# KLab/YAIK

Hardware: AMD Instinct MI355X
Metric: Mpix/s tile encode (alpha reject + 7 gradient passes + 8x8 range quant), 8K RGBA (higher is better)
Workload: dtype u8/int32 (+f32 mode-selection sums)

## Files before the change

### yaik_amd/csrc/yk_stages.hip

```cpp
#include "yk_common.h"
#ifdef YK_TEST_HOOKS
#include "../../include/yaik_hip_test.h"
#endif
#include "yk_device.h"

typedef int yk_i4 __attribute__((ext_vector_type(4)));
#ifndef YK_ALPHA_WAVES
#define YK_ALPHA_WAVES 3
#endif
__global__ __launch_bounds__(64 * YK_ALPHA_WAVES, 4) void yk_alpha_kernel(const int32_t* __restrict__ alpha0, int strideElems, int w, int h, int y0,
                                                      uint8_t* __restrict__ keep0, int mtW, int mtH, unsigned long long planeStride,
                                                      unsigned long long keepStride, yk_i4* __restrict__ unitBox0, unsigned total) {
    const int lane = threadIdx.x & 63;
    const int vecPerRow = w >> 2;
    const int nSeg = (vecPerRow + 63) >> 6;
    const int nUnits = nSeg * ((mtH + YK_ALPHA_R - 1) / YK_ALPHA_R);
    const unsigned uu = blockIdx.x * YK_ALPHA_WAVES + (threadIdx.x >> 6);
    if (uu >= total) return;
    const int f = (int)(uu / (unsigned)nUnits), u = (int)(uu - (unsigned)f * (unsigned)nUnits);
    const int32_t* alpha = alpha0 + (size_t)f * planeStride;
    uint8_t* keep = keep0 + (size_t)f * keepStride;
    const int tyU = u / nSeg, seg = u - tyU * nSeg, ty0 = tyU * YK_ALPHA_R;
    const int xv = seg * 64 + lane;
    const bool inX = xv < vecPerRow;
    const bool tileLane = (lane & 3) == 0;
    const int tx = xv >> 2;
    const int xvc = min(xv, vecPerRow - 1);
    uint32_t nzBits = 0, undBits = 0, rowsLeft = 0;
    {
        yk_i4 p[YK_ALPHA_R][2];
#pragma unroll
        for (int r = 0; r < YK_ALPHA_R; r++) {
            const int yA = min((ty0 + r) * 16, h - 1), yB = min(yA + 15, h - 1);
            p[r][0] = __builtin_nontemporal_load(reinterpret_cast<const yk_i4*>(alpha + (size_t)yA * strideElems + (size_t)xvc * 4));
            p[r][1] = __builtin_nontemporal_load(reinterpret_cast<const yk_i4*>(alpha + (size_t)yB * strideElems + (size_t)xvc * 4));
        }
#pragma unroll
        for (int r = 0; r < YK_ALPHA_R; r++) {
            const bool on = inX && (ty0 + r) * 16 < h;
            const yk_i4 o = p[r][0] | p[r][1];
            const bool nz = ((o.x | o.y | o.z | o.w) != 0) & on;
            const unsigned long long pb = __ballot(nz);
            const bool und = on && ((pb >> (lane & ~3)) & 0xFULL) == 0;
            nzBits |= (nz ? 1u : 0u) << r; undBits |= (und ? 1u : 0u) << r;
            if (__ballot(und) != 0) rowsLeft |= 1u << r;
        }
    }
    while (rowsLeft) {
        const int rA = __ffs((int)rowsLeft) - 1; rowsLeft &= rowsLeft - 1;
        const bool two = rowsLeft != 0;
        const int rB = two ? __ffs((int)rowsLeft) - 1 : rA; rowsLeft &= rowsLeft - 1;
        yk_i4 a[2][14];
#pragma unroll
        for (int j = 0; j < 2; j++) {
            const int r = j ? rB : rA, ty = ty0 + r;
            const bool und = (j == 0 || two) && ((undBits >> r) & 1u) != 0;
            const int32_t* col = alpha + (size_t)(ty * 16) * strideElems + (size_t)xv * 4;
#pragma unroll
            for (int k = 0; k < 14; k++) {
                a[j][k] = (yk_i4){0, 0, 0, 0};
                if (und && ty * 16 + 1 + k < h) a[j][k] = __builtin_nontemporal_load(reinterpret_cast<const yk_i4*>(col + (size_t)(1 + k) * strideElems));
            }
        }
#pragma unroll
        for (int j = 0; j < 2; j++) {
            int m = 0;
#pragma unroll
            for (int k = 0; k < 14; k++) m |= a[j][k].x | a[j][k].y | a[j][k].z | a[j][k].w;
            nzBits |= (m != 0 ? 1u : 0u) << (j ? rB : rA);
        }
    }
    int colLo = 0x7FFFFFFF, colHi = -1, rowLo = 0x7FFFFFFF, rowHi = -1;
#pragma unroll
    for (int r = 0; r < YK_ALPHA_R; r++) {
        const int ty = ty0 + r;
        if (ty >= mtH) break;
        const unsigned long long b = __ballot(((nzBits >> r) & 1u) != 0);
        const bool kept = ((b >> (lane & ~3)) & 0xFULL) != 0;
        if (tileLane && tx < mtW) keep[(size_t)ty * mtW + tx] = kept ? 1 : 0;
        const unsigned long long kb64 = __ballot(tileLane && kept && tx < mtW);
        if (kb64) {
            colLo = min(colLo, seg * 16 + ((__ffsll((long long)kb64) - 1) >> 2));
            colHi = max(colHi, seg * 16 + ((63 - __clzll((long long)kb64)) >> 2));
            rowLo = min(rowLo, ty); rowHi = max(rowHi, ty);
        }
    }
    if (lane == 0) {
        const bool any = colHi >= 0;
        unitBox0[(size_t)f * nUnits + u] = any ? (yk_i4){colLo * 16, y0 + rowLo * 16, colHi * 16 + 16, y0 + rowHi * 16 + 16} : (yk_i4){9999999, 9999999, -1, -1};
    }
}

__global__ __launch_bounds__(256) void yk_alpha_box_kernel(const yk_i4* __restrict__ unitBox0, int nUnits, int32_t* __restrict__ bounds) {
    __shared__ yk_i4 s_box[4];
    const int lane = threadIdx.x & 63, wv = threadIdx.x >> 6;
    const yk_i4* ub = unitBox0 + (size_t)blockIdx.x * nUnits;
    int x0 = 9999999, gy0 = 9999999, x1 = -1, gy1 = -1;
    for (int base = 0; base < nUnits; base += 256 * 16) {
        yk_i4 v[16];
#pragma unroll
        for (int j = 0; j < 16; j++) v[j] = ub[min(base + j * 256 + (int)threadIdx.x, nUnits - 1)];
#pragma unroll
        for (int j = 0; j < 16; j++) { x0 = min(x0, v[j].x); gy0 = min(gy0, v[j].y); x1 = max(x1, v[j].z); gy1 = max(gy1, v[j].w); }
    }
#pragma unroll
    for (int d = 1; d < 64; d <<= 1) {
        x0 = min(x0, __shfl_xor(x0, d)); x1 = max(x1, __shfl_xor(x1, d));
        gy0 = min(gy0, __shfl_xor(gy0, d)); gy1 = max(gy1, __shfl_xor(gy1, d));
    }
    if (lane == 0) s_box[wv] = (yk_i4){x0, gy0, x1, gy1};
    __syncthreads();
    if (threadIdx.x == 0) {
#pragma unroll
        for (int k = 1; k < 4; k++) { x0 = min(x0, s_box[k].x); gy0 = min(gy0, s_box[k].y); x1 = max(x1, s_box[k].z); gy1 = max(gy1, s_box[k].w); }
        *reinterpret_cast<yk_i4*>(bounds + (size_t)blockIdx.x * 16 + 8) = (yk_i4){x0, gy0, x1, gy1};
    }
}

__global__ void yk_alpha_publish_kernel(int32_t* __restrict__ bounds, int srcOff, int fullW, int fullH) {
    bounds += (size_t)blockIdx.x * 16;
    const int b0 = bounds[srcOff], b1 = bounds[srcOff + 1], b2 = bounds[srcOff + 2], b3 = bounds[srcOff + 3];
    bounds[0] = b0; bounds[1] = b1; bounds[2] = b2; bounds[3] = b3;
    bounds[4] = (b0 == 0 && b1 == 0 && b2 == fullW && b3 == fullH) ? 1 : 0;
}

#define YK_SCAN_TILE 1024

__global__ __launch_bounds__(1024) void yk_scan1_kernel(const uint8_t* __restrict__ tileCount, size_t T8, uint32_t* __restrict__ blockCnt) {
    __shared__ uint32_t s_tmp[32];
    const size_t i = (size_t)blockIdx.x * YK_SCAN_TILE + threadIdx.x;
    const uint32_t c = (i < T8) ? tileCount[i] : 0;
    uint32_t tot2, totN;
    yk_block_exscan(c ? 1u : 0u, s_tmp, &tot2);
    yk_block_exscan(c, s_tmp, &totN);
    if (threadIdx.x == 0) { blockCnt[(size_t)blockIdx.x * 2] = totN; blockCnt[(size_t)blockIdx.x * 2 + 1] = tot2; }
}

__device__ __forceinline__ void yk_scan2_body(uint32_t* __restrict__ blockCnt, uint32_t* __restrict__ blockSums, int nBlocks, uint32_t* __restrict__ totals, uint32_t* s_tmp) {
    uint32_t baseN = 0, baseD = 0;
    for (int start = 0; start < nBlocks; start += 1024) {
        const int i = start + threadIdx.x;
        const uint32_t n = i < nBlocks ? blockCnt[i * 2] : 0, d = i < nBlocks ? blockCnt[i * 2 + 1] : 0;
        uint32_t totN, totD;
        const uint32_t en = yk_block_exscan(n, s_tmp, &totN);
        const uint32_t ed = yk_block_exscan(d, s_tmp, &totD);
        if (i < nBlocks) {
            blockSums[i * 2] = baseN + en; blockSums[i * 2 + 1] = baseD + ed;
            blockCnt[i * 2] = 0; blockCnt[i * 2 + 1] = 0;
        }
        baseN += totN; baseD += totD;
    }
    if (threadIdx.x < 3) { totals[threadIdx.x * 2] = baseD; totals[threadIdx.x * 2 + 1] = baseN; }
}
__global__ __launch_bounds__(1024) void yk_scan2_kernel(uint32_t* __restrict__ blockCnt, uint32_t* __restrict__ blockSums, int nBlocks,
                                                        uint32_t* __restrict__ totals, unsigned long long blockNStride) {
    __shared__ uint32_t s_tmp[32];
    yk_scan2_body(blockCnt + (size_t)blockIdx.x * blockNStride, blockSums + (size_t)blockIdx.x * blockNStride, nBlocks, totals + (size_t)blockIdx.x * 8, s_tmp);
}

__global__ __launch_bounds__(1024) void yk_scan1r_kernel(const uint32_t* __restrict__ runSums, unsigned long long runStride, int nRuns,
                                                         uint32_t* __restrict__ blockCnt, unsigned long long blockNStride, int nBlocks,
                                                         const uint8_t* __restrict__ bm0b, unsigned long long bm0bStride, uint8_t* __restrict__ bitmap0,
                                                         unsigned long long bitmap0Stride, int nB64) {
    const size_t f = blockIdx.y;
    const int g = (int)blockIdx.x * 1024 + (int)threadIdx.x;
    if (runSums) {
        const uint4* rs4 = reinterpret_cast<const uint4*>(runSums + f * runStride);
        const int n4 = (nRuns + 3) >> 2;
        const uint4 v = g < n4 ? rs4[g] : make_uint4(0u, 0u, 0u, 0u);
        uint32_t acc = v.x + v.y + v.z + v.w;
        acc += __shfl_xor(acc, 16, 32); acc += __shfl_xor(acc, 8, 32); acc += __shfl_xor(acc, 4, 32); acc += __shfl_xor(acc, 2, 32); acc += __shfl_xor(acc, 1, 32);
        const int blk = g >> 5;
        if ((threadIdx.x & 31) == 0 && blk < nBlocks) {
            uint2* dst = reinterpret_cast<uint2*>(blockCnt + f * blockNStride) + blk;
            *dst = make_uint2(16u * (acc & 0xFFFFu), acc >> 16);
        }
    }
    if (g < nB64) {
        const uint32_t b = reinterpret_cast<const uint32_t*>(bm0b + f * bm0bStride)[g];
        uint16_t* dst = reinterpret_cast<uint16_t*>(bitmap0 + f * bitmap0Stride);
        dst[g] = (uint16_t)((b & 0xFu) | ((b >> 4) & 0xF0u) | ((b >> 8) & 0xF00u) | ((b >> 12) & 0xF000u));
        if (g == nB64 - 1 && (nB64 & 1)) dst[nB64] = 0;
    }
}

struct __attribute__((aligned(8))) YkPiece16 { uint32_t a, b, c, d; };
__global__ __launch_bounds__(256) void yk_pack_kernel(const uint8_t* __restrict__ tileCount, const uint16_t* __restrict__ tileDef, const uint2* __restrict__ tileInfo,
                                                      const uint8_t* __restrict__ slots, size_t T8, const uint32_t* __restrict__ blockSums, int nBlocks,
                                                      uint16_t* __restrict__ defsOut, uint32_t* __restrict__ nibOut, size_t nibStrideWords, YkFrameStrides fs,
                                                      const uint32_t* __restrict__ blockCnt, uint32_t* __restrict__ totals) {
    __shared__ uint32_t s_wave[4];
    __shared__ unsigned long long s_pre;
    __shared__ uint32_t s_off[YK_SCAN_TILE];
    __shared__ uint8_t s_cnt[YK_SCAN_TILE];
    {
        const size_t f = blockIdx.z;
        tileCount += f * fs.tileCount; tileDef += f * fs.tileDef; slots += f * fs.slots; blockSums += f * fs.blockN;
        if (tileInfo) tileInfo += f * fs.tileInfo;
        defsOut += f * fs.defsOut; nibOut += f * (fs.nibOut / 4);
        if (blockCnt) { blockCnt += f * fs.blockN; totals += f * 8; }
    }
    const int lane = threadIdx.x & 63, wave = threadIdx.x >> 6;
    const size_t i0 = (size_t)blockIdx.x * YK_SCAN_TILE, i = i0 + (size_t)threadIdx.x * 4;
    uint32_t c[4] = {0, 0, 0, 0}, d01[4] = {0, 0, 0, 0}, d2[4] = {0, 0, 0, 0};
    if (tileInfo && i + 4 <= T8) {
        const uint4 r0 = reinterpret_cast<const uint4*>(tileInfo + i)[0], r1 = reinterpret_cast<const uint4*>(tileInfo + i)[1];
        d01[0] = r0.x; c[0] = r0.y >> 16; d2[0] = r0.y & 0xFFFFu; d01[1] = r0.z; c[1] = r0.w >> 16; d2[1] = r0.w & 0xFFFFu;
        d01[2] = r1.x; c[2] = r1.y >> 16; d2[2] = r1.y & 0xFFFFu; d01[3] = r1.z; c[3] = r1.w >> 16; d2[3] = r1.w & 0xFFFFu;
    } else {
#pragma unroll
        for (int j = 0; j < 4; j++) {
            if (i + j >= T8) continue;
            if (tileInfo) { const uint2 ti = tileInfo[i + j]; c[j] = ti.y >> 16; d01[j] = ti.x; d2[j] = ti.y & 0xFFFFu; }
            else { c[j] = tileCount[i + j]; if (c[j]) { d01[j] = (uint32_t)tileDef[i + j] | ((uint32_t)tileDef[T8 + i + j] << 16); d2[j] = tileDef[2 * T8 + i + j]; } }
        }
    }
    if (blockCnt && wave == 3) {
        unsigned long long acc = 0;
        for (int k = lane; k < (int)blockIdx.x; k += 64) { const uint2 v = reinterpret_cast<const uint2*>(blockCnt)[k]; acc += ((unsigned long long)v.y << 32) | v.x; }
#pragma unroll
        for (int d = 1; d < 64; d <<= 1) acc += __shfl_xor(acc, d);
        if (lane == 0) s_pre = acc;
    }
    uint32_t w[4], mine = 0;
#pragma unroll
    for (int j = 0; j < 4; j++) { w[j] = mine; mine += c[j] | (c[j] ? 0x10000u : 0u); }
    uint32_t incl = mine;
#pragma unroll
    for (int d = 1; d < 64; d <<= 1) { const uint32_t o = __shfl_up(incl, d); if (lane >= d) incl += o; }
    if (lane == 63) s_wave[wave] = incl;
    __syncthreads();
    uint32_t front = incl - mine;
#pragma unroll
    for (int k = 0; k < 3; k++) if (k < wave) front += s_wave[k];
    uint32_t baseN, baseD;
    if (blockCnt) {
        baseN = (uint32_t)s_pre; baseD = (uint32_t)(s_pre >> 32);
        if (blockIdx.x == (unsigned)nBlocks - 1 && threadIdx.x < 3) {
            const uint2 v = reinterpret_cast<const uint2*>(blockCnt)[nBlocks - 1];
            totals[threadIdx.x * 2] = baseD + v.y; totals[threadIdx.x * 2 + 1] = baseN + v.x;
        }
    } else { baseN = blockSums[(size_t)blockIdx.x * 2]; baseD = blockSums[(size_t)blockIdx.x * 2 + 1]; }
#pragma unroll
    for (int j = 0; j < 4; j++) {
        const uint32_t e = front + w[j], en = e & 0xFFFFu, ed = e >> 16;
        s_off[threadIdx.x * 4 + j] = (baseN + en) >> 1;
        s_cnt[threadIdx.x * 4 + j] = (uint8_t)c[j];
        if (c[j]) { defsOut[baseD + ed] = (uint16_t)d01[j]; defsOut[T8 + baseD + ed] = (uint16_t)(d01[j] >> 16); defsOut[2 * T8 + baseD + ed] = (uint16_t)d2[j]; }
    }
    __syncthreads();
    const int half = threadIdx.x & 1;
#pragma unroll
    for (int p = 0; p < 3; p++) {
        uint8_t* out = reinterpret_cast<uint8_t*>(nibOut + (size_t)p * nibStrideWords);
#pragma unroll
        for (int it = 0; it < 8; it++) {
            const int t = it * 128 + (threadIdx.x >> 1);
            const size_t ti = i0 + t;
            const int left = (s_cnt[t] >> 1) - half * 16;
            const uint8_t* src = slots + ((size_t)p * T8 + ti) * YK_SLOT + half * 16;
            uint8_t* dst = out + s_off[t] + half * 16;
            if (left >= 16) { const uint4 v = *reinterpret_cast<const uint4*>(src); *reinterpret_cast<YkPiece16*>(dst) = YkPiece16{v.x, v.y, v.z, v.w}; }
            else if (left >= 8) *reinterpret_cast<uint2*>(dst) = *reinterpret_cast<const uint2*>(src);
        }
    }
}

static int (*g_crossCheckLauncher)(hipStream_t, const YkEncodeParams*) = nullptr;
#ifdef YK_TEST_HOOKS
extern "C" int yk_set_cross_check_launcher(void* fn) { g_crossCheckLauncher = reinterpret_cast<int (*)(hipStream_t, const YkEncodeParams*)>(fn); return YK_OK; }
#endif

int yk_launch_alpha(yk_ctx* c, bool batch) {
    const int F = batch ? c->nFrames : 1;
    const YkFrameView V = yk_frame(c, batch ? 0 : c->curFrame);
    const long long nUnits = (long long)yk_alpha_units(c->fullW, c->mtH);
    if (nUnits * F > 0x7FFFFFFFLL) return yk_fail(c, YK_ERR_BAD_ARG, "too many alpha work units for one launch");
    yk_i4* unitBox = reinterpret_cast<yk_i4*>(static_cast<int*>(c->img.alphaUnitBox));
    hipLaunchKernelGGL(yk_alpha_kernel, dim3((unsigned)((nUnits * F + YK_ALPHA_WAVES - 1) / YK_ALPHA_WAVES)), dim3(64 * YK_ALPHA_WAVES), 0, c->stream, V.plane[3], c->strideElems,
                       c->fullW, c->h, c->y0, V.keep, c->mtW, c->mtH, (unsigned long long)c->fs.plane, (unsigned long long)c->fs.keep, unitBox, (unsigned)(nUnits * F));
    hipLaunchKernelGGL(yk_alpha_box_kernel, dim3((unsigned)F), dim3(256), 0, c->stream, unitBox, (int)nUnits, V.bounds);
    YK_HIP(c, hipGetLastError());
    c->boundsOff = 8;
    return YK_OK;
}

int yk_launch_alpha_finish(yk_ctx* c, const int32_t* globalBBox) {
    if (globalBBox) {
        int32_t b[5] = { globalBBox[0], globalBBox[1], globalBBox[2], globalBBox[3], 0 };
        b[4] = (b[0] == 0 && b[1] == 0 && b[2] == c->fullW && b[3] == c->fullH) ? 1 : 0;
        YK_HIP(c, hipMemcpyAsync(yk_frame(c).bounds, b, sizeof b, hipMemcpyHostToDevice, c->stream));
        c->boundsOff = 0;
    }
    return YK_OK;
}

int yk_launch_encode(yk_ctx* c, int rejectFactor, int mode3BitOnly, int wantDst, bool batch) {
    const YkFrameView V = yk_frame(c, batch ? 0 : c->curFrame);
    YkEncodeParams P;
    for (int i = 0; i < 4; i++) P.plane[i] = V.plane[i];
    P.strideElems = c->strideElems; P.w = c->fullW; P.h = c->h; P.hAvail = c->h + c->halo; P.y0 = c->y0; P.fullH = c->fullH;
    P.rejectFactor = rejectFactor; P.startMode = mode3BitOnly ? 3 : 0; P.wantDst = wantDst; P.ablate = c->ablate;
    P.keep = (c->nPlanes == 4) ? V.keep : nullptr;
    P.bounds = (c->nPlanes == 4) ? V.bounds + c->boundsOff : nullptr;
    for (int i = 0; i < 7; i++) P.bitmap[i] = V.bitmap[i];
    P.coverage = V.coverage; P.tileDef = V.tileDef; P.tileCount = V.tileCount; P.slots = V.slots;
    P.blockCnt = c->kernelVersion == 2 ? V.blockCnt : nullptr;
    for (int i = 0; i < 3; i++) P.dst[i] = c->img.dst[i];
    P.tilesW = c->tilesW; P.tilesH = c->tilesH; P.mtW = c->mtW; P.mtH = c->mtH;
    P.xBB64 = (c->fullW + 63) / 64; P.yBB64 = (c->h + 63) / 64; P.xBB32 = (c->fullW + 31) / 32; P.yBB32 = (c->h + 31) / 32;
    P.nFrames = batch ? c->nFrames : 1; P.fs = c->fs;
    P.qtab = c->qtab;
    P.small = V.small;
    auto off = [&](const void* p) { return (uint32_t)(static_cast<const uint8_t*>(p) - V.small); };
    for (int i = 0; i < 7; i++) P.oBm[i] = off(V.bitmap[i]);
    P.oBm0b = off(V.bm0b); P.oCov = off(V.coverage); P.oInfo = off(V.tileInfo); P.oRun = off(V.runSums);
    P.divXBB64 = c->divXBB64; P.divNBf = c->divNBf;
    P.outTab = c->img.outTab; P.outFrame0 = batch ? 0u : (uint32_t)c->curFrame;
    P.pixCache = nullptr; c->pixCacheValid = false;
    if (c->pixCacheOn && !batch && c->kernelVersion == 2 && c->nFrames == 1) {
        if (!c->img.pixCache) YK_HIP(c, c->img.pixCache.alloc(c->stream, (size_t)P.xBB64 * 64 * ((size_t)(c->h + 15) / 16 * 16) / 4, 4096));
        P.pixCache = c->img.pixCache; c->pixCacheValid = true;
    }
    if (c->kernelVersion == 2) return yk_launch_encode2(c, P);
    if (batch) return yk_fail(c, YK_ERR_STATE, "batches need kernel version 2");
    if (c->nPlanes == 4) {
        hipLaunchKernelGGL(yk_alpha_publish_kernel, dim3(1), dim3(1), 0, c->stream, V.bounds, c->boundsOff, c->fullW, c->fullH);
        P.bounds = V.bounds;
    }
    if (!g_crossCheckLauncher) return yk_fail(c, YK_ERR_STATE, "kernel version 1 is not part of this library: register it with yk_set_cross_check_launcher");
    if (g_crossCheckLauncher(c->stream, &P) != 0) return yk_fail(c, YK_ERR_HIP, "cross-check kernel launch", hipGetLastError());
    return YK_OK;
}

int yk_launch_pack(yk_ctx* c, bool batch) {
    const size_t T8 = (size_t)c->tilesW * c->tilesH;
    const int nb = c->nScanBlocks, F = batch ? c->nFrames : 1;
    const YkFrameView V = yk_frame(c, batch ? 0 : c->curFrame);
    if (c->kernelVersion != 2) hipLaunchKernelGGL(yk_scan1_kernel, dim3(nb), dim3(1024), 0, c->stream, V.tileCount, T8, V.blockCnt);
    const bool v2 = c->kernelVersion == 2;
    const uint32_t* runSums = (v2 && (c->tilesW & 7) == 0) ? V.runSums : nullptr;
    const uint8_t* bm0b = v2 ? V.bm0b : nullptr;
    const uint2* tileInfo = v2 ? V.tileInfo : nullptr;
    const int nB64 = ((c->fullW + 63) / 64) * ((c->h + 63) / 64);
    if (v2) {
        const int nRuns = (int)((T8 + 7) / 8), n4 = (nRuns + 3) >> 2;
        const int items = runSums ? (n4 > nB64 ? n4 : nB64) : nB64;
        hipLaunchKernelGGL(yk_scan1r_kernel, dim3((unsigned)((items + 1023) / 1024), F), dim3(1024), 0, c->stream, runSums, (unsigned long long)c->fs.runSums, nRuns,
                           V.blockCnt, (unsigned long long)c->fs.blockN, nb, bm0b, (unsigned long long)c->fs.bm0b,
                           V.bitmap[0], (unsigned long long)c->fs.bitmap[0], nB64);
    }
    if (!runSums) hipLaunchKernelGGL(yk_scan2_kernel, dim3(F), dim3(1024), 0, c->stream, V.blockCnt, V.blockSums, nb, V.totals, (unsigned long long)c->fs.blockN);
    hipLaunchKernelGGL(yk_pack_kernel, dim3(nb, 1, F), dim3(256), 0, c->stream, V.tileCount, V.tileDef, tileInfo,
                       V.slots, T8, V.blockSums, nb, V.defsOut, reinterpret_cast<uint32_t*>(V.nibOut), c->nibStride / 4, c->fs,
                       runSums ? V.blockCnt : (const uint32_t*)nullptr, V.totals);
    YK_HIP(c, hipGetLastError());
    return YK_OK;
}

__global__ void yk_selftest_div_kernel(int* mismatches) {
    const int n = blockIdx.x, d = threadIdx.x + 1;
    const float fn = (float)n, fd = (float)d;
    const float ref = __fdiv_rn(fn, fd);
    const float got = yk_div_exact(fn, fd, __fdiv_rn(1.0f, fd));
    if (__float_as_uint(ref) != __float_as_uint(got)) atomicAdd(mismatches, 1);
}

__global__ void yk_selftest_scale_kernel(int* mismatches) {
    const int scale = blockIdx.x + 1, d8 = threadIdx.x;
    if (d8 < 32) return;
    const int dnum = (d8 - 32) * 127 + (scale - 1);
    const int ref = dnum / scale;
    const int got = __float2int_rz(((float)dnum + 0.5f) * __builtin_amdgcn_rcpf((float)scale));
    if (ref != got) atomicAdd(mismatches, 1);
}

__global__ void yk_selftest_r1div_kernel(int* mismatches) {
    const int n = blockIdx.x * 16 + (threadIdx.x >> 4), d0 = (threadIdx.x & 15) * 16;
    for (int k = 0; k < 16; k++) {
        const int d = d0 + k;
        if (d < 1 || d > 255) continue;
        const int got = __float2int_rz(((float)n + 0.5f) * __builtin_amdgcn_rcpf((float)d));
        if (got != n / d) atomicAdd(mismatches, 1);
    }
}

__global__ void yk_selftest_r1magic_kernel(int* mismatches) {
    const int delta = blockIdx.x, x = threadIdx.x;
    if (x > delta) return;
    for (int minCol = 0; minCol + delta <= 255; minCol++) {
        uint32_t A, B;
        yk_r1_magic(delta, minCol, &A, &B);
        const int v = minCol + x;
        int idx = 0;
        if (delta) { const int n = (v - minCol) * 15 + (delta >> 1) - 1; idx = n < 0 ? -1 : n / delta; }
        const uint32_t got = (__umul24((uint32_t)v, A) + B) >> 20;
        if (got != (uint32_t)(1 + idx)) atomicAdd(mismatches, 1);
    }
}

#ifdef YK_TEST_HOOKS
extern "C" int yk_selftest(yk_ctx* c, int which, int* result) {
    if (!c || !result) return YK_ERR_BAD_ARG;
    YK_HIP(c, hipSetDevice(c->device));
    YkBuf<int> d;
    YK_HIP(c, d.alloc(c->stream, 1));
    YK_HIP(c, hipMemsetAsync(d, 0, sizeof(int), c->stream));
    if (which == 0) hipLaunchKernelGGL(yk_selftest_div_kernel, dim3(256), dim3(256), 0, c->stream, d);
    else if (which == 1) hipLaunchKernelGGL(yk_selftest_scale_kernel, dim3(256), dim3(256), 0, c->stream, d);
    else if (which == 2) hipLaunchKernelGGL(yk_selftest_r1div_kernel, dim3(256), dim3(256), 0, c->stream, d);
    else if (which == 3) yk_selftest_qtab_launch(c, d);
    else if (which == 4) hipLaunchKernelGGL(yk_selftest_r1magic_kernel, dim3(256), dim3(256), 0, c->stream, d);
    else return yk_fail(c, YK_ERR_BAD_ARG, "unknown selftest");
    YK_HIP(c, hipMemcpyAsync(result, d, sizeof(int), hipMemcpyDeviceToHost, c->stream));
    YK_HIP(c, hipStreamSynchronize(c->stream));
    return YK_OK;
}
#endif
```

Measured before the change: 240,300.

## Compact coded tiles in pack kernel and batch slot loads for memory-level parallelism

The pack kernel now builds a compacted list of coded tiles in shared memory (offset plus tile index and count), so threads iterate only over real work items instead of every tile. Loads for several items are issued together before a waitcnt, then stored, to keep more memory requests in flight. Optional nontemporal load and store paths are added behind macros. Profiling scripts for the pack kernel are also added. The cost is more registers per thread and a loop over the compacted item list.

```diff
diff --git a/profiles/pack_in_flight/pack_frames.py b/profiles/pack_in_flight/pack_frames.py
--- /dev/null
+++ b/profiles/pack_in_flight/pack_frames.py
@@ -0,0 +1,26 @@
+import os, sys
+sys.path.insert(0, os.path.dirname(os.path.dirname(os.path.dirname(os.path.abspath(__file__)))))
+import torch
+from yaik_amd.encoder import HipTileEncoder
+
+reps, classes = int(sys.argv[1]), sys.argv[2:]
+W = 8192
+dev = "cuda"
+enc = HipTileEncoder(0)
+for name in classes:
+    if name == "noise":
+        g = torch.Generator(device=dev); g.manual_seed(1)
+        img = torch.randint(0, 256, (3, W, W), device=dev, generator=g)
+    elif name == "ramp":
+        x = torch.arange(W, device=dev, dtype=torch.int64)[None, :].expand(W, W)
+        y = torch.arange(W, device=dev, dtype=torch.int64)[:, None].expand(W, W)
+        img = torch.stack([(255 * x) // W, (255 * y) // W, (255 * (x + y)) // (2 * W)])
+    else:
+        raise SystemExit(f"unknown class {name}")
+    planes = img.to(torch.int32).contiguous()
+    enc.set_image(planes)
+    for _ in range(reps + 2):
+        enc.encode(3, False, False)
+    defs, _, nn = enc.range_streams(0)
+    print(f"class {name}: {nn} nibbles per plane, coded tiles {defs.size} of {W * W // 64}", flush=True)
+enc.close()
diff --git a/profiles/pack_in_flight/summarize.py b/profiles/pack_in_flight/summarize.py
--- /dev/null
+++ b/profiles/pack_in_flight/summarize.py
@@ -0,0 +1,48 @@
+import csv, glob, os, runpy, statistics, sys
+
+mode, d = sys.argv[1], sys.argv[2]
+S, E = (lambda r: int(r["Start_Timestamp"])), (lambda r: int(r["End_Timestamp"]))
+
+
+def kernel_rows(pattern):
+    rows = []
+    for f in glob.glob(f"{d}/**/*kernel_trace.csv", recursive=True):
+        rows += [r for r in csv.DictReader(open(f)) if pattern(r["Kernel_Name"])]
+    rows.sort(key=S)
+    return rows
+
+
+def line(label, us, mb):
+    med = statistics.median(us)
+    rate = f"  {mb:.1f} MB / median = {mb / med:.2f} TB/s" if mb else ""
+    print(f"{label}: yk_pack_kernel min {min(us):6.1f} us  median {med:6.1f} us  max {max(us):6.1f} us  ({len(us)} launches){rate}")
+
+
+if mode == "bench":
+    label, mb = sys.argv[3], float(sys.argv[4])
+    pack = kernel_rows(lambda n: "yk_pack_kernel" in n)
+    sel = pack[len(pack) // 4: len(pack) * 3 // 4]
+    line(label, [(E(r) - S(r)) / 1e3 for r in sel], mb)
+elif mode == "classes":
+    reps, classes = int(sys.argv[3]), [a.split(":") for a in sys.argv[4:]]
+    pack = kernel_rows(lambda n: "yk_pack_kernel" in n)
+    per = reps + 2
+    assert len(pack) == per * len(classes), (len(pack), per, classes)
+    for i, (name, mb) in enumerate(classes):
+        line(f"all-{name} 8192^2 RGB frame, alone", [(E(r) - S(r)) / 1e3 for r in pack[i * per + 2:(i + 1) * per]], float(mb))
+elif mode == "timeline":
+    sys.argv = [os.path.join(os.path.dirname(os.path.abspath(__file__)), "..", "event_chain", "summarize.py"), "timeline", d]
+    runpy.run_path(sys.argv[0], run_name="__main__")
+    rows = kernel_rows(lambda n: "yk_pack_kernel" in n or "encode2" in n)
+    fused = [r for r in rows if "encode2" in r["Kernel_Name"]]
+    lo, hi = S(fused[len(fused) // 4]), S(fused[len(fused) * 3 // 4])
+    st, en, dur = [], [], []
+    for r in rows:
+        if "yk_pack_kernel" not in r["Kernel_Name"] or not lo <= S(r) <= hi:
+            continue
+        other = min(fused, key=lambda f: abs(S(f) - S(r)))
+        st.append((S(r) - S(other)) / 1e3); en.append((E(r) - S(other)) / 1e3); dur.append((E(r) - S(r)) / 1e3)
+    print(f"\npack kernel, {len(st)} frames: starts {statistics.mean(st):+.1f} us (min {min(st):+.1f}, max {max(st):+.1f}) and ends {statistics.mean(en):+.1f} us "
+          f"(min {min(en):+.1f}, max {max(en):+.1f}) relative to the START of the other frame's fused kernel; duration mean {statistics.mean(dur):.1f} us  median {statistics.median(dur):.1f}")
+else:
+    raise SystemExit(f"unknown mode {mode}")
diff --git a/yaik_amd/csrc/yk_stages.hip b/yaik_amd/csrc/yk_stages.hip
--- a/yaik_amd/csrc/yk_stages.hip
+++ b/yaik_amd/csrc/yk_stages.hip
@@ -184,7 +184,18 @@
     }
 }
 
-struct __attribute__((aligned(8))) YkPiece16 { uint32_t a, b, c, d; };
+#ifndef YK_PACK_DEPTH
+#define YK_PACK_DEPTH 8
+#endif
+#ifndef YK_PACK_PLANES
+#define YK_PACK_PLANES 1
+#endif
+#ifndef YK_PACK_NT
+#define YK_PACK_NT 0
+#endif
+typedef uint32_t yk_u4 __attribute__((ext_vector_type(4)));
+typedef uint32_t yk_u2 __attribute__((ext_vector_type(2)));
+typedef yk_u4 yk_u4s __attribute__((aligned(8)));
 __global__ __launch_bounds__(256) void yk_pack_kernel(const uint8_t* __restrict__ tileCount, const uint16_t* __restrict__ tileDef, const uint2* __restrict__ tileInfo,
                                                       const uint8_t* __restrict__ slots, size_t T8, const uint32_t* __restrict__ blockSums, int nBlocks,
                                                       uint16_t* __restrict__ defsOut, uint32_t* __restrict__ nibOut, size_t nibStrideWords, YkFrameStrides fs,
@@ -192,7 +203,7 @@
     __shared__ uint32_t s_wave[4];
     __shared__ unsigned long long s_pre;
     __shared__ uint32_t s_off[YK_SCAN_TILE];
-    __shared__ uint8_t s_cnt[YK_SCAN_TILE];
+    __shared__ uint16_t s_tile[YK_SCAN_TILE];
     {
         const size_t f = blockIdx.z;
         tileCount += f * fs.tileCount; tileDef += f * fs.tileDef; slots += f * fs.slots; blockSums += f * fs.blockN;
@@ -244,24 +255,54 @@
 #pragma unroll
     for (int j = 0; j < 4; j++) {
         const uint32_t e = front + w[j], en = e & 0xFFFFu, ed = e >> 16;
-        s_off[threadIdx.x * 4 + j] = (baseN + en) >> 1;
-        s_cnt[threadIdx.x * 4 + j] = (uint8_t)c[j];
-        if (c[j]) { defsOut[baseD + ed] = (uint16_t)d01[j]; defsOut[T8 + baseD + ed] = (uint16_t)(d01[j] >> 16); defsOut[2 * T8 + baseD + ed] = (uint16_t)d2[j]; }
+        if (c[j]) {
+            s_off[ed] = (baseN + en) >> 1;
+            s_tile[ed] = (uint16_t)((threadIdx.x * 4 + j) | ((c[j] >> 4) << 10));
+            defsOut[baseD + ed] = (uint16_t)d01[j]; defsOut[T8 + baseD + ed] = (uint16_t)(d01[j] >> 16); defsOut[2 * T8 + baseD + ed] = (uint16_t)d2[j];
+        }
     }
     __syncthreads();
-    const int half = threadIdx.x & 1;
-#pragma unroll
-    for (int p = 0; p < 3; p++) {
-        uint8_t* out = reinterpret_cast<uint8_t*>(nibOut + (size_t)p * nibStrideWords);
-#pragma unroll
-        for (int it = 0; it < 8; it++) {
-            const int t = it * 128 + (threadIdx.x >> 1);
-            const size_t ti = i0 + t;
-            const int left = (s_cnt[t] >> 1) - half * 16;
-            const uint8_t* src = slots + ((size_t)p * T8 + ti) * YK_SLOT + half * 16;
-            uint8_t* dst = out + s_off[t] + half * 16;
-            if (left >= 16) { const uint4 v = *reinterpret_cast<const uint4*>(src); *reinterpret_cast<YkPiece16*>(dst) = YkPiece16{v.x, v.y, v.z, v.w}; }
-            else if (left >= 8) *reinterpret_cast<uint2*>(dst) = *reinterpret_cast<const uint2*>(src);
+    const uint32_t nItems = 2u * ((s_wave[0] >> 16) + (s_wave[1] >> 16) + (s_wave[2] >> 16) + (s_wave[3] >> 16));
+    for (uint32_t first = 0; first < nItems; first += 256u * YK_PACK_DEPTH) {
+        int left[YK_PACK_DEPTH];
+        uint32_t dstOff[YK_PACK_DEPTH];
+        size_t srcOff[YK_PACK_DEPTH];
+#pragma unroll
+        for (int k = 0; k < YK_PACK_DEPTH; k++) {
+            const uint32_t item = first + (uint32_t)k * 256u + threadIdx.x, half = item & 1u;
+            left[k] = 0; dstOff[k] = 0; srcOff[k] = 0;
+            if (item < nItems) {
+                const uint32_t e = s_tile[item >> 1];
+                left[k] = (int)(e >> 10) * 8 - (int)half * 16;
+                dstOff[k] = s_off[item >> 1] + half * 16;
+                srcOff[k] = (i0 + (e & 1023u)) * YK_SLOT + half * 16;
+            }
+        }
+#pragma unroll
+        for (int p0 = 0; p0 < 3; p0 += YK_PACK_PLANES) {
+            yk_u4 v[YK_PACK_PLANES][YK_PACK_DEPTH];
+#pragma unroll
+            for (int q = 0; q < YK_PACK_PLANES; q++)
+#pragma unroll
+                for (int k = 0; k < YK_PACK_DEPTH; k++) {
+                    const yk_u4* src = reinterpret_cast<const yk_u4*>(slots + (size_t)(p0 + q) * T8 * YK_SLOT + srcOff[k]);
+                    v[q][k] = (yk_u4){0u, 0u, 0u, 0u};
+                    if (left[k] >= 8) v[q][k] = (YK_PACK_NT & 1) ? __builtin_nontemporal_load(src) : *src;
+                }
+            __builtin_amdgcn_s_waitcnt(0x0F70);
+#pragma unroll
+            for (int q = 0; q < YK_PACK_PLANES; q++) {
+                uint8_t* out = reinterpret_cast<uint8_t*>(nibOut + (size_t)(p0 + q) * nibStrideWords);
+#pragma unroll
+                for (int k = 0; k < YK_PACK_DEPTH; k++) {
+                    uint8_t* dst = out + dstOff[k];
+                    if (left[k] >= 16) {
+                        if (YK_PACK_NT & 2) __builtin_nontemporal_store(v[q][k], reinterpret_cast<yk_u4s*>(dst)); else *reinterpret_cast<yk_u4s*>(dst) = v[q][k];
+                    } else if (left[k] >= 8) {
+                        if (YK_PACK_NT & 2) __builtin_nontemporal_store(v[q][k].xy, reinterpret_cast<yk_u2*>(dst)); else *reinterpret_cast<yk_u2*>(dst) = v[q][k].xy;
+                    }
+                }
+            }
         }
     }
 }
```

Measured after the change: 243,300 (median of 6 runs). 1.2% higher.
